# ArnauGabrielAtienza/pytorch_distributed_examples

Hardware: AMD Instinct MI355X
Metric: images/sec (whole node) MNIST DDP + ResNet50 RPC-MP at 1/2/4/8 MI355X (higher is better)
Workload: dtype bf16; 1 GPU; model=mnist_cnn_Net, global_batch=1024, image=1x28x28, parallelism=dp1, hipgraph=True, fused_step=True, rccl_nranks=1, steps_per_graph=5, allreduce=none

## Files before the change

### csrc/kernels/cnn_fused.hip

```cpp
#include <cstddef>
#include <type_traits>

#include "adasum_weights.h"
#include "common.cuh"
#include "optim_device.h"
#include "pde_kernels.h"
#include "xgmi_device.h"

namespace pde {

namespace {

constexpr int T = 1024;
constexpr int NW = T / 64;
constexpr int NI = 4;
constexpr int C1 = 10, C2 = 20, KS = 5, H0 = 28, O1 = 24, P1 = 12, O2 = 8, P2 = 4, F1 = 50, F2 = 10;
constexpr int NX = H0 * H0, NC1 = P1 * P1, NR1 = C1 * NC1, NC2 = P2 * P2, NIN = C2 * NC2;
constexpr int RP16 = 146, RP8 = 148;
static_assert(RP16 >= NC1 && RP8 >= NC1, "channel planes hold the 144 cells");
static_assert(RP16 % 2 == 0 && RP8 % 4 == 0, "P9 reads 4 cells' argmax bytes as one aligned 4-byte word");
constexpr int EP = 148;
constexpr unsigned char AM_DEAD = 0xFF;
constexpr int XP = 36, NXP = H0 * XP;
constexpr int DHP = 52;
// ... 8 lines not shown
constexpr int D2N_P = 24, D2N_RP = 264, D2N_Q = 128;
constexpr int D2N_IM = 7 * D2N_RP + 7 * D2N_P + 2 * D2N_Q + 8;
static_assert(D2N_IM % 8 == 0 && D2N_P % 8 == 0 && D2N_RP % 8 == 0 && D2N_Q % 8 == 0, "d2n: 16-byte slots");
__host__ __device__ constexpr int d2n_ofs(int im, int y, int x, int co) {
  return im * D2N_IM + y * D2N_RP + x * D2N_P + (co >> 3) * D2N_Q + (co & 7);
}
constexpr int D2R = O2 * O2 + 8;
constexpr int MT1 = O1 * O1 / 16;
constexpr int MTD = NC1 * 1 / 16;
constexpr int KSW1 = O1 * O1 / 32;
struct KsRange {
  int lo, hi;
};
__host__ __device__ constexpr bool p7b_tap_live(int cls, int r, int ky, int kx) {
  const int pos = cls * 16 + r, y = pos / P1 - ky, x = pos % P1 - kx;
  return y >= 0 && y < O2 && x >= 0 && x < O2;
}
__host__ __device__ constexpr KsRange p7b_ks_range(int cls) {
  int lo = KSD, hi = 0;
  for (int r = 0; r < 16; ++r)
    for (int ky = 0; ky < KS; ++ky)
      for (int kx = 0; kx < KS; ++kx) {
        if (!p7b_tap_live(cls, r, ky, kx)) continue;
        const int g0 = (ky * KS + kx) * CG, k0 = g0 / 4, k1 = (g0 + CG - 1) / 4;
        lo = k0 < lo ? k0 : lo;
        hi = k1 + 1 > hi ? k1 + 1 : hi;
      }
  return {lo, hi};
}
__host__ __device__ constexpr bool p7b_range_covers(int cls, KsRange q) {
  for (int g = 0; g < NGD; ++g)
    for (int r = 0; r < 16; ++r)
      if (p7b_tap_live(cls, r, g / CG / KS, g / CG % KS) && (g / 4 < q.lo || g / 4 >= q.hi)) return false;
  return q.lo >= 0 && q.hi <= KSD;
}
__host__ __device__ constexpr bool p7b_ranges_ok() {
  int sum = 0;
  for (int c = 0; c < MTD; ++c) {
    if (!p7b_range_covers(c, p7b_ks_range(c))) return false;
    sum += p7b_ks_range(c).hi - p7b_ks_range(c).lo;
  }
  return sum == 126;
}
constexpr bool ks_is(KsRange q, int lo, int hi) { return q.lo == lo && q.hi == hi; }
static_assert(MTD == 9 && NC1 % 16 == 0 && p7b_ranges_ok(), "conv2 dgrad: every live tap inside its class's range");
static_assert(ks_is(p7b_ks_range(0), 0, 7) && ks_is(p7b_ks_range(1), 0, 12) && ks_is(p7b_ks_range(2), 0, 15) &&
                  ks_is(p7b_ks_range(3), 0, KSD) && ks_is(p7b_ks_range(4), 0, KSD) &&
                  ks_is(p7b_ks_range(5), 0, KSD) && ks_is(p7b_ks_range(6), 3, KSD) &&
                  ks_is(p7b_ks_range(7), 7, KSD) && ks_is(p7b_ks_range(8), 12, KSD),
              "conv2 dgrad k-step ranges (rows 0-1, 1-2, 2-3, 4..7, 8-9, 9-10, 10-11)");
__host__ __device__ constexpr uint64_t p7b_pack(bool hi) {
  uint64_t v = 0;
  for (int c = 0; c < MTD; ++c)
    v |= static_cast<uint64_t>(hi ? p7b_ks_range(c).hi : p7b_ks_range(c).lo) << (5 * c);
  return v;
}
constexpr uint64_t P7B_LO = p7b_pack(false), P7B_HI = p7b_pack(true);
static_assert(KSD < 32 && MTD * 5 <= 64, "5-bit fields");
constexpr int P7B_WCLS[NW] = {3, 4, 5, 5, 3, 4, 6, 6, 1, 7, 2, 2, 1, 7, 0, 0};
constexpr int P7B_WPAIR[NW] = {0, 0, 0, 1, 1, 1, 0, 1, 0, 0, 0, 1, 1, 1, 0, 1};
__host__ __device__ constexpr int p7b_wave_steps(int w) {
  const int c = P7B_WCLS[w];
  int n = p7b_ks_range(c).hi - p7b_ks_range(c).lo;
  if (c == 0) n += p7b_ks_range(MTD - 1).hi - p7b_ks_range(MTD - 1).lo;
  return 2 * n;
}
__host__ __device__ constexpr bool p7b_map_ok() {
  for (int c = 0; c < MTD - 1; ++c) {
    int n[2] = {0, 0};
    for (int w = 0; w < NW; ++w)
      if (P7B_WCLS[w] == c) ++n[P7B_WPAIR[w]];
    if (n[0] != 1 || n[1] != 1) return false;
  }
  int tot = 0;
  for (int s = 0; s < 4; ++s) {
    int n = 0;
    for (int w = s; w < NW; w += 4) n += p7b_wave_steps(w);
    if (n < 120 || n > 132) return false;
    tot += n;
  }
  return tot == NI * 126;
}
static_assert(NW == 16 && NI == 4 && p7b_map_ok(), "conv2 dgrad wave map: complete, balanced over the SIMDs");
__host__ __device__ constexpr uint64_t p7b_pack_map(bool pair) {
  uint64_t v = 0;
  for (int w = 0; w < NW; ++w) v |= static_cast<uint64_t>(pair ? P7B_WPAIR[w] : P7B_WCLS[w]) << (4 * w);
  return v;
}
constexpr uint64_t P7B_MCLS = p7b_pack_map(false), P7B_MPAIR = p7b_pack_map(true);
constexpr int XMAP_P7B_FULLK = 8;
constexpr int O_W1 = 0, O_B1 = O_W1 + W1N, O_W2 = O_B1 + C1, O_B2 = O_W2 + W2N, O_FC1W = O_B2 + C2,
              O_FC1B = O_FC1W + FC1N, O_FC2W = O_FC1B + F1, O_FC2B = O_FC2W + FC2N, NPARAM = O_FC2B + F2;
constexpr int NSLAB = NPARAM - FC1N;
static_assert(O_W2 % 4 == 0 && C2 % 4 == 0 && W2N % 4 == 0, "W2T: float4 columns of 4 co");
constexpr int SLAB_OFS = (32 - O_W2 % 32) % 32;
constexpr int NSLABP = (SLAB_OFS + NSLAB + 31) / 32 * 32;
constexpr int S_FC1B = O_FC1B - FC1N, S_FC2W = O_FC2W - FC1N, S_FC2B = O_FC2B - FC1N;
constexpr int NACT = F1 + NIN;
__host__ __device__ constexpr int act_pitch(int nwg) { return (nwg * NI + 7) & ~7; }
static_assert(O_FC1W % 4 == 0 && FC1N % 4 == 0 && NSLAB % 4 == 0, "float4 slab columns");

__device__ __forceinline__ float hash_u01(unsigned long long seed, unsigned long long id) {
  unsigned long long z = seed + 0x9E3779B97F4A7C15ULL * (id + 1);
  z = (z ^ (z >> 30)) * 0xBF58476D1CE4E5B9ULL;
  z = (z ^ (z >> 27)) * 0x94D049BB133111EBULL;
  z ^= z >> 31;
  return static_cast<float>(z >> 40) * (1.0f / 16777216.0f);
}

__device__ __forceinline__ f32x4 mfma(const u16x8& a, const u16x8& b, const f32x4& c) {
  return __builtin_amdgcn_mfma_f32_16x16x32_bf16(__builtin_bit_cast(bf16x8, a), __builtin_bit_cast(bf16x8, b), c, 0,
                                                 0, 0);
}

template <int CTRL>
__device__ __forceinline__ float dppf(float v) {
  return __builtin_bit_cast(float, __builtin_amdgcn_update_dpp(0, __builtin_bit_cast(int, v), CTRL, 0xF, 0xF, false));
}
__device__ __forceinline__ float lanef(float v, int l) {
  return __builtin_bit_cast(float, __builtin_amdgcn_readlane(__builtin_bit_cast(int, v), l));
}
constexpr int DPP_XOR1 = 0xB1, DPP_XOR2 = 0x4E, DPP_HALF_MIRROR = 0x141, DPP_MIRROR = 0x140;
template <class Op>
__device__ __forceinline__ float wave_all(float v, Op op) {
  v = op(v, dppf<DPP_XOR1>(v));
  v = op(v, dppf<DPP_XOR2>(v));
  v = op(v, dppf<DPP_HALF_MIRROR>(v));
  v = op(v, dppf<DPP_MIRROR>(v));
  return op(op(lanef(v, 0), lanef(v, 16)), op(lanef(v, 32), lanef(v, 48)));
}
__device__ __forceinline__ float wave_sum_dpp(float v) { return wave_all(v, [](float a, float b) { return a + b; }); }
__device__ __forceinline__ float wave_max_dpp(float v) { return wave_all(v, [](float a, float b) { return fmaxf(a, b); }); }

struct CnnSmem {
  alignas(16) uint16_t r1n[NI][NC1][C1P];
  alignas(16) u16x8 w2f[KS2][2][64];
  alignas(16) u16x8 w2d[KSD][64];
  alignas(16) u16x8 w1f[64];
  alignas(16) uint16_t d2n[NI * D2N_IM];
  alignas(16) uint16_t d2[NI][C2][D2R];
  alignas(16) uint16_t zero16[8];
  alignas(8) uint32_t p7tab[KSD * 4][2];
  uint16_t x[NI][NXP];
  uint16_t xpad[18];
  uint16_t x1[NI][NXP];
  uint16_t xonepad[48];
  alignas(16) uint16_t xone[NI][NXP];
  alignas(16) uint16_t r1[NI][C1 * RP16];
  alignas(16) float b1[C1];
  alignas(16) float b2[C2];
  alignas(16) float fc1b[F1];
  alignas(16) float fc2w[FC2N];
  alignas(16) float fc2b[F2];
  alignas(16) float r2[NI][NIN];
  alignas(16) float dp2[NI][NIN];
  float h1[NI][F1], m1[NI][F1], h1d[NI][F1];
  alignas(16) float dh[NI][DHP];
  float mc2[NI][C2];
  float logit[NI][F2], dlog[NI][F2];
  float lossim[NI];
  float valid[NI];
  int label[NI];
  alignas(16) unsigned char a1[NI][C1 * RP8];
  unsigned char a2[NI][NIN];
};
static_assert(sizeof(CnnSmem) <= 160 * 1024, "LDS budget");
static_assert((offsetof(CnnSmem, xone) - offsetof(CnnSmem, x)) / 4 % 32 == 4,
              "xone bank offset from x (P9 B reads: scripts/p9_lds_model.py; x1's: cnn_p1)");
static_assert(offsetof(CnnSmem, w2f) == offsetof(CnnSmem, r1n) + sizeof(uint16_t) * NI * NC1 * C1P &&
                  sizeof(uint32_t) * NI * C1 * EP <= sizeof(uint16_t) * NI * NC1 * C1P + sizeof(u16x8) * KS2 * 2 * 64,
              "e1 aliases r1n + w2f");
static_assert(offsetof(CnnSmem, d2n) == offsetof(CnnSmem, w1f) + sizeof(u16x8) * 64 &&
                  NW * 2 * 64 * sizeof(f32x4) <= sizeof(u16x8) * (KSD * 64 + 64) + sizeof(uint16_t) * NI * D2N_IM,
              "P9 partials alias w2d + w1f + d2n (not e1)");
static_assert(offsetof(CnnSmem, w2d) == offsetof(CnnSmem, w2f) + sizeof(u16x8) * KS2 * 2 * 64, "w2f, w2d adjacent");
constexpr int NT2 = 16 / NW;
constexpr int NFRAG = KS2 * 2 * 64 + KSD * 64 + 64;
constexpr int NF2F = KS2 * 2 * 64, NF2D = KSD * 64;
static_assert(NF2F <= 2 * T && NF2D <= 2 * T && NF2F + NF2D + 64 == NFRAG, "fragment slots");
static_assert(offsetof(CnnSmem, w1f) == offsetof(CnnSmem, w2d) + sizeof(u16x8) * KSD * 64, "w2d, w1f adjacent");
constexpr int FC1_KC = NIN / 32;
constexpr int DP2_JC = 3;
constexpr int DP2_J = 16;
static_assert(F1 - DP2_J * (DP2_JC - 1) <= 20 && DP2_J % 4 == 0 && DHP >= DP2_J * (DP2_JC - 1) + 20, "dp2 chunks");
static_assert(F1 * FC1_KC <= T && NIN * DP2_JC <= T, "fc1 work split");
static_assert(sizeof(float) * NI * NIN * DP2_JC <= sizeof(u16x8) * KS2 * 2 * 64, "dp2 partials alias w2f");
static_assert(NT2 * NW == 16, "conv2 wgrad tiling");

__device__ __forceinline__ void lds_sync() {
  __builtin_amdgcn_fence(__ATOMIC_RELEASE, "workgroup", "local");
  __builtin_amdgcn_s_barrier();
  __builtin_amdgcn_fence(__ATOMIC_ACQUIRE, "workgroup", "local");
}

__device__ __forceinline__ uint32_t lds_addr(const void* p) {
#if defined(__HIP_DEVICE_COMPILE__)
  return (uint32_t)(const __attribute__((address_space(3))) unsigned char*)(p);
#else
  return static_cast<uint32_t>(reinterpret_cast<uintptr_t>(p));
#endif
}
__device__ __forceinline__ u16x8 lds_read16(uint32_t o) {
#if defined(__HIP_DEVICE_COMPILE__)
  return *(const __attribute__((address_space(3))) u16x8*)(o);
#else
  return u16x8{static_cast<uint16_t>(o), 0, 0, 0, 0, 0, 0, 0};
#endif
}

struct CnnTail {
  const float* gscale;
  float* grads;
  float* loss;
  unsigned long long* rng;
  float* params;
  const float* hp;
  uint16_t* frag;
  int* step;
  unsigned* bar;
  int* err;
  int accumulate, B, on, pad;
};
__device__ void cnn_fused_tail(const CnnTail& tl, int rb, f32x4* part, uint32_t* s_epoch, int* s_fail,
                               const float* slabs, int nwg, const uint16_t* acts, const float* loss_part);

__device__ __forceinline__ void cnn_grid_barrier(unsigned* bar, unsigned n, int* err, unsigned* s_gen) {
  asm volatile("s_waitcnt vmcnt(0)" ::: "memory");
  __syncthreads();
  if (threadIdx.x == 0) {
    const unsigned g0 = __hip_atomic_load(bar + 1, __ATOMIC_RELAXED, __HIP_MEMORY_SCOPE_AGENT);
    __builtin_amdgcn_fence(__ATOMIC_RELEASE, "agent");
    const unsigned old = __hip_atomic_fetch_add(bar, 1u, __ATOMIC_RELAXED, __HIP_MEMORY_SCOPE_AGENT);
    if (old == n - 1) {
      __hip_atomic_store(bar, 0u, __ATOMIC_RELAXED, __HIP_MEMORY_SCOPE_AGENT);
      __hip_atomic_fetch_add(bar + 1, 1u, __ATOMIC_RELEASE, __HIP_MEMORY_SCOPE_AGENT);
    } else {
      const uint64_t t0 = __builtin_amdgcn_s_memrealtime();
      while (__hip_atomic_load(bar + 1, __ATOMIC_RELAXED, __HIP_MEMORY_SCOPE_AGENT) == g0) {
        if (__builtin_amdgcn_s_memrealtime() - t0 > 200000000ull) {
          __hip_atomic_store(err, 1, __ATOMIC_RELAXED, __HIP_MEMORY_SCOPE_AGENT);
          break;
        }
        __builtin_amdgcn_s_sleep(1);
      }
    }
    __builtin_amdgcn_fence(__ATOMIC_ACQUIRE, "agent");
    *s_gen = g0;
  }
  __syncthreads();
}

template <int SM>
__device__ __forceinline__ void out_st(float* p, float v) {
  if constexpr (SM == 1) __builtin_nontemporal_store(v, p);
  else if constexpr (SM == 2) asm volatile("global_store_dword %0, %1, off sc1" ::"v"(p), "v"(v) : "memory");
  else *p = v;
}
template <int SM>
__device__ __forceinline__ void out_st_u16x4(uint16_t* p, u16x4 v) {
  if constexpr (SM == 1) __builtin_nontemporal_store(v, reinterpret_cast<u16x4*>(p));
  else st_vec(reinterpret_cast<u16x4*>(p), v, SM >= 2);
}
template <int SM>
__device__ __forceinline__ void out_st4(float* p, f32x4 v) {
  if constexpr (SM == 1) __builtin_nontemporal_store(v, reinterpret_cast<f32x4*>(p));
  else if constexpr (SM >= 2) asm volatile("global_store_dwordx4 %0, %1, off sc1" ::"v"(p), "v"(v) : "memory");
  else *reinterpret_cast<f32x4*>(p) = v;
}

template <bool TRAIN, class Smem>
__device__ __forceinline__ void cnn_p0(Smem& S, int t, int n0, int B, const float* __restrict__ images,
                                       const int64_t* __restrict__ tgt, const float* __restrict__ params,
                                       const u16x8* __restrict__ frag, const unsigned long long* __restrict__ rng,
                                       float p_drop2, float p_drop1, int training, u16x8 (&fr)[2]) {
  static_assert(NI * NX / 4 <= T, "one image quad per thread");
  constexpr int NH = C1 + C2 + F1 + FC2N + F2;
  static_assert(NH <= T && O_FC2W == O_FC1B + F1 && O_FC2B == O_FC2W + FC2N, "fc1b, fc2w, fc2b contiguous");
  static_assert(offsetof(Smem, fc2b) == offsetof(Smem, fc2w) + sizeof(float) * FC2N, "fc2w, fc2b adjacent");
  static_assert((NI & (NI - 1)) == 0 && 384 % NI == 0, "label threads 384..: slot t & (NI - 1)");
  const int qi = min(t, NI * NX / 4 - 1);
  const int qim = (qi * 4) / NX, qoff = qi * 4 - qim * NX;
  const int hi = min(t, NH - 1);
  const int hsrc = hi < C1 ? O_B1 + hi : hi < C1 + C2 ? O_B2 + hi - C1 : O_FC1B + hi - (C1 + C2);
  const int lslot = t & (NI - 1);
  const int64_t* lbase = tgt != nullptr ? tgt : reinterpret_cast<const int64_t*>(frag);
  const int lidx = tgt != nullptr ? min(n0 + lslot, B - 1) : 0;
  int rofs = 0;
  asm("" : "+v"(rofs));
  const u16x8 fw1 = frag[NF2F + NF2D + (t & 63)];
  const f32x4 img = *reinterpret_cast<const f32x4*>(images + static_cast<long>(min(n0 + qim, B - 1)) * NX + qoff);
  const float hv = params[hsrc];
  unsigned long long r0 = 0;
  if constexpr (TRAIN) r0 = rng[rofs];
  const int lab = reinterpret_cast<const int*>(lbase)[2 * lidx];
  fr[0] = frag[t];
  fr[1] = frag[min(t + T, NF2F - 1)];
  static_assert(H0 % 4 == 0 && XP >= H0 + 6, "image quads within a row; kx = 5 reads stay in the row");
  for (int i = t; i < NI * H0 * (XP - H0 + 1); i += T) {
    const int r = i / (XP - H0 + 1), c = i - r * (XP - H0 + 1);
    if (c > 0) (&S.x[0][0])[r * XP + H0 - 1 + c] = 0;
    (&S.x1[0][0])[r * XP + H0 - 1 + c] = 0;
  }
  if constexpr (TRAIN) {
    for (int i = t; i < NI * O2 * O2; i += T) {
      const int im = i / (O2 * O2), pos = i - im * (O2 * O2);
      *reinterpret_cast<u16x8*>(&S.d2n[d2n_ofs(im, pos / O2, pos % O2, 16)]) = u16x8{0, 0, 0, 0, 0, 0, 0, 0};
    }
    if (t < 8) S.zero16[t] = 0;
    static_assert((NI * NXP) % 8 == 0 && NI * NXP / 8 <= T, "xone: one 16-byte store per thread");
    if (t < NI * NXP / 8)
      reinterpret_cast<u16x8*>(&S.xone[0][0])[t] =
          u16x8{0x3F80, 0x3F80, 0x3F80, 0x3F80, 0x3F80, 0x3F80, 0x3F80, 0x3F80};
    if (t < KSD * 4) {
      const int g = t, tap = g / CG, cg = g - tap * CG, ky = tap / KS, kx = tap - ky * KS;
      S.p7tab[g][0] = g < NGD ? (static_cast<uint32_t>(ky) << 16) | static_cast<uint32_t>(kx) : 0x80008000u;
      S.p7tab[g][1] = static_cast<uint32_t>(g < NGD ? (-(ky * D2N_RP + kx * D2N_P) + cg * D2N_Q) * 2 : 0);
    }
  }
  if (t < 64) S.w1f[t] = fw1;
  if (t < NI * NX / 4) {
    const int im = qim, off = qoff, n = n0 + im;
    const f32x4 v = n < B ? img : f32x4{0.f, 0.f, 0.f, 0.f};
    const int row = off / H0, col = off - row * H0;
    uint16_t* dst = &S.x[im][row * XP + col];
    const uint16_t b0 = f2bf(v[0]), b1 = f2bf(v[1]), b2 = f2bf(v[2]), b3 = f2bf(v[3]);
    dst[0] = b0; dst[1] = b1; dst[2] = b2; dst[3] = b3;
    uint16_t* d1 = &S.x1[im][row * XP + col];
    if (col > 0) d1[-1] = b0;
    d1[0] = b1; d1[1] = b2; d1[2] = b3;
  }
  if (t < NH) {
    const int hofs = hi < C1             ? static_cast<int>(offsetof(Smem, b1)) + 4 * hi
                     : hi < C1 + C2      ? static_cast<int>(offsetof(Smem, b2)) + 4 * (hi - C1)
                     : hi < C1 + C2 + F1 ? static_cast<int>(offsetof(Smem, fc1b)) + 4 * (hi - (C1 + C2))
                                         : static_cast<int>(offsetof(Smem, fc2w)) + 4 * (hi - (C1 + C2 + F1));
    *reinterpret_cast<float*>(reinterpret_cast<unsigned char*>(&S) + hofs) = hv;
  }
  if constexpr (TRAIN) {
    const unsigned long long seed = r0 * 0xD1B54A32D192ED03ULL;
    const float keep2 = training ? 1.f / (1.f - p_drop2) : 1.f;
    const float keep1 = training ? 1.f / (1.f - p_drop1) : 1.f;
    if (t < NI * C2) {
      const int im = t / C2, c = t - im * C2;
      const unsigned long long id = static_cast<unsigned long long>(n0 + im) * C2 + c;
      S.mc2[im][c] = (!training || hash_u01(seed ^ 0x5bd1e995ULL, id) >= p_drop2) ? keep2 : 0.f;
    } else if (t >= 128 && t < 128 + NI * F1) {
      const int u = t - 128, im = u / F1, j = u - im * F1;
      const unsigned long long id = static_cast<unsigned long long>(n0 + im) * F1 + j;
      S.m1[im][j] = (!training || hash_u01(seed ^ 0x27d4eb2fULL, id) >= p_drop1) ? keep1 : 0.f;
    }
  }
  if (t >= 384 && t < 384 + NI) {
    const bool ok = tgt != nullptr && n0 + lslot < B;
    if constexpr (TRAIN) S.valid[lslot] = ok ? 1.f : 0.f;
    S.label[lslot] = ok ? static_cast<int>(lab) : 0;
  }
}


__device__ __forceinline__ float pool4(const f32x4& v, int& am) {
  am = 0;
  float m = v[0];
  if (v[1] > m) { m = v[1]; am = 1; }
  if (v[2] > m) { m = v[2]; am = 2; }
  if (v[3] > m) { m = v[3]; am = 3; }
  return m;
}

static_assert(P1 % 4 == 0 && MT1 * 4 == NC1, "conv1 tiles: 4 cells of one row");
static_assert((NI * MT1) % NW == 0, "every wave runs the same number of conv1 tiles");
constexpr int NT1 = NI * MT1 / NW;
constexpr int P1_TR = P1 / 4;
static_assert(MT1 % NT1 == 0, "conv1: a wave's tiles lie in one image");
static_assert(NT1 % P1_TR == 0, "conv1: a wave's tiles are whole cell rows");
constexpr int P1_WI = MT1 / NT1;
constexpr int P1_WR = NT1 / P1_TR;
struct P1Tile {
  int im, py, px0;
};
__host__ __device__ constexpr P1Tile p1_tile(int w, int u) {
  return {w / P1_WI, (w % P1_WI) * P1_WR + u / P1_TR, (u % P1_TR) * 4};
}
__host__ __device__ constexpr bool p1_map_ok() {
  for (int tile = 0; tile < NI * MT1; ++tile) {
    int n = 0;
    for (int w = 0; w < NW; ++w)
      for (int u = 0; u < NT1; ++u) {
        const P1Tile q = p1_tile(w, u);
        if (q.im < 0 || q.im >= NI || q.py < 0 || q.py >= P1 || q.px0 < 0 || q.px0 + 4 > P1) return false;
        if (q.im * MT1 + q.py * P1_TR + q.px0 / 4 == tile) ++n;
      }
    if (n != 1) return false;
  }
  return true;
}
static_assert(p1_map_ok(), "conv1 wave map: the 16 waves cover each of the NI * MT1 tiles exactly once");

template <bool TRAIN, class Smem>
__device__ __forceinline__ void cnn_p1(Smem& S, int lane, int wid) {
  static_assert((offsetof(Smem, x1) - offsetof(Smem, x)) / 4 % 32 == 9, "x1 bank offset from x (P1 gathers)");
  const int lr = lane & 15, lg = lane >> 4;
  int koff[4];
#pragma unroll
  for (int p = 0; p < 4; ++p) {
    const int k = lg * 8 + 2 * p;
    koff[p] = k < KS * 6 ? (k / 6) * XP + (k % 6) : 0;
  }
  const u16x8 bw = S.w1f[lane];
  const int tap = lr & 3, dy = tap >> 1, dx = tap & 1;
  const uint16_t* xsrc = dx ? &S.x1[0][0] - 1 : &S.x[0][0];
  const P1Tile w0 = p1_tile(wid, 0);
  const uint16_t* xlane = xsrc + dy * XP + 2 * (lr >> 2) + dx + w0.im * NXP + 2 * w0.py * XP;
  const uint16_t* xb[4];
#pragma unroll
  for (int p = 0; p < 4; ++p) xb[p] = xlane + koff[p];
  u16x8 ag[NT1];
#pragma unroll
  for (int u = 0; u < NT1; ++u) {
    const P1Tile q = p1_tile(0, u);
    const int xo = 2 * q.py * XP + 2 * q.px0;
    u32x4 v;
#pragma unroll
    for (int p = 0; p < 4; ++p) v[p] = *reinterpret_cast<const uint32_t*>(xb[p] + xo);
    ag[u] = __builtin_bit_cast(u16x8, v);
  }
  f32x4 accs[NT1];
#pragma unroll
  for (int u = 0; u < NT1; ++u) accs[u] = mfma(ag[u], bw, f32x4{0.f, 0.f, 0.f, 0.f});
  const int co = lr;
  const float b1v = S.b1[min(co, C1 - 1)];
  const float bias1 = co < C1 ? b1v : 0.f;
  const int cw = w0.py * P1 + lg;
  uint16_t* r1n = &S.r1n[w0.im][cw][co];
  uint16_t rr[NT1];
  int am[NT1];
#pragma unroll
  for (int u = 0; u < NT1; ++u) {
    const P1Tile q = p1_tile(0, u);
    const float m = pool4(accs[u], am[u]);
    rr[u] = f2bf(fmaxf(m + bias1, 0.f));
    r1n[(q.py * P1 + q.px0) * C1P] = rr[u];
    if constexpr (TRAIN) {
      if (rr[u] == 0) am[u] = AM_DEAD;
      asm volatile("" : "+v"(am[u]));
    }
  }
  if constexpr (TRAIN) {
    if (co < C1) {
      uint16_t* r1 = &S.r1[w0.im][co * RP16 + cw];
      unsigned char* a1 = &S.a1[w0.im][co * RP8 + cw];
#pragma unroll
      for (int u = 0; u < NT1; ++u) {
        const P1Tile q = p1_tile(0, u);
        r1[q.py * P1 + q.px0] = rr[u];
        a1[q.py * P1 + q.px0] = static_cast<unsigned char>(am[u]);
      }
    }
  }
}

template <class Smem>
__device__ __forceinline__ void cnn_store_w2f(Smem& S, int t, const u16x8 (&fr)[2]) {
  u16x8* dst = &S.w2f[0][0][0];
  dst[t] = fr[0];
  if (t + T < NF2F) dst[t + T] = fr[1];
}

__device__ __forceinline__ void cnn_fc1_rows(int t, const float* __restrict__ gFC1W, f32x4 (&w3)[8]) {
  if (t < F1 * FC1_KC) {
    const int j = t / FC1_KC, kc = t - j * FC1_KC;
    const f32x4* w4 = reinterpret_cast<const f32x4*>(gFC1W + j * NIN + kc * 4);
#pragma unroll
    for (int q = 0; q < 8; ++q) w3[q] = w4[q * (FC1_KC)];
  }
}

template <bool TRAIN, class Smem>
__device__ __forceinline__ void cnn_p2(Smem& S, int lane, int wid) {
  const int lr = lane & 15, lg = lane >> 4;
  for (int mtile = wid; mtile < NI * 4; mtile += NW) {
    const int im = mtile >> 2, mt = mtile & 3;
    const int tap = lr & 3, dy = tap >> 1, dx = tap & 1;
    const int cell = mt * 4 + (lr >> 2), py = cell >> 2, px = cell & 3;
    const int rb = (2 * py + dy) * P1 + 2 * px + dx;
    f32x4 acc0 = {0.f, 0.f, 0.f, 0.f}, acc1 = acc0;
    const uint16_t* r1n = &S.r1n[im][0][(lg & 1) * 8];
#pragma unroll
    for (int ks = 0; ks < KS2; ++ks) {
      const int tp = 2 * ks + (lg >> 1), ky = tp / KS, kx = tp - ky * KS;
      const u16x8 a = tp < KS * KS ? *reinterpret_cast<const u16x8*>(r1n + (rb + ky * P1 + kx) * C1P)
                                   : u16x8{0, 0, 0, 0, 0, 0, 0, 0};
      acc0 = mfma(a, S.w2f[ks][0][lane], acc0);
      acc1 = mfma(a, S.w2f[ks][1][lane], acc1);
    }
#pragma unroll
    for (int nt = 0; nt < 2; ++nt) {
      const int co = nt * 16 + lr;
      if (co < C2) {
        int am;
        const float m = pool4(nt == 0 ? acc0 : acc1, am);
        const int q = co * NC2 + mt * 4 + lg;
        if constexpr (TRAIN) {
          S.r2[im][q] = fmaxf((m + S.b2[co]) * S.mc2[im][co], 0.f);
          S.a2[im][q] = static_cast<unsigned char>(am);
        } else {
          S.r2[im][q] = fmaxf(m + S.b2[co], 0.f);
        }
      }
    }
  }
}

template <bool TRAIN, class Smem>
__device__ __forceinline__ void cnn_p3(Smem& S, int t, const f32x4 (&w3)[8]) {
  static_assert(sizeof(float) * NI * F1 * FC1_KC <= sizeof(Smem::w2f), "fc1 partials alias w2f");
  float* part = reinterpret_cast<float*>(&S.w2f[0][0][0]);
  if (t < F1 * FC1_KC) {
    const int j = t / FC1_KC, kc = t - j * FC1_KC;
    const f32x4* w = w3;
    float s4[NI] = {0.f, 0.f, 0.f, 0.f};
#pragma unroll
    for (int q = 0; q < 8; ++q)
#pragma unroll
      for (int im = 0; im < NI; ++im) {
        const f32x4 x = *reinterpret_cast<const f32x4*>(&S.r2[im][q * 4 * FC1_KC + kc * 4]);
        s4[im] += w[q][0] * x[0] + w[q][1] * x[1] + w[q][2] * x[2] + w[q][3] * x[3];
      }
#pragma unroll
    for (int im = 0; im < NI; ++im) part[(kc * NI + im) * F1 + j] = s4[im];
  }
  lds_sync();
  if (t < NI * F1) {
    const int im = t / F1, j = t - im * F1;
    float s1 = S.fc1b[j];
#pragma unroll
    for (int kc = 0; kc < FC1_KC; ++kc) s1 += part[(kc * NI + im) * F1 + j];
    const float h = fmaxf(s1, 0.f);
    S.h1[im][j] = h;
    if constexpr (TRAIN) S.h1d[im][j] = h * S.m1[im][j];
  }
}

struct CnnHead {
  float logit;
  float lse;
  float ly;
  int y;
};
template <class Smem>
__device__ __forceinline__ CnnHead cnn_head(const Smem& S, const float* h, int im, int lane) {
  static_assert(4 * F2 <= 64, "P4: a lane quad per logit");
  const int v = lane >> 2, p = lane & 3;
  const bool lv = v < F2;
  const int vr = lv ? v : 0;
  float s = 0.f;
#pragma unroll
  for (int k = 0; k < (F1 + 3) / 4; ++k) {
    const int j = p + 4 * k;
    if (j < F1) s += S.fc2w[vr * F1 + j] * h[j];
  }
  s += dppf<DPP_XOR1>(s);
  s += dppf<DPP_XOR2>(s);
  const float logit = s + S.fc2b[vr];
  const float m = wave_max_dpp(lv ? logit : -INFINITY);
  const float ex = __expf(logit - m);
  const float se = wave_sum_dpp(lv && p == 0 ? ex : 0.f);
  const float lse = m + __logf(se);
  const int y = S.label[im];
  const float ly = lanef(logit, __builtin_amdgcn_readfirstlane(4 * y));
  return {logit, lse, ly, y};
}

template <int SM, bool BREG>
__global__ __launch_bounds__(T) void k_cnn_train(const float* __restrict__ images, const int64_t* __restrict__ tgt,
                                                 int B, const float* __restrict__ params,
                                                 const u16x8* __restrict__ frag,
                                                 const unsigned long long* __restrict__ rng, float p_drop2,
                                                 float p_drop1, int training, float* __restrict__ slabs,
                                                 float* __restrict__ loss_part, uint16_t* __restrict__ acts,
                                                 unsigned long long* __restrict__ stamps, int stop_after,
                                                 CnnTail tail, int xmap) {
#define PDE_STAMP(k)                                                                      \
  if (stamps != nullptr && threadIdx.x == 0) stamps[blockIdx.x * 16 + (k)] = wall_clock64(); \
  if (stop_after == (k)) return
  asm volatile("" ::"s"(images), "s"(tgt), "s"(B), "s"(params), "s"(frag), "s"(rng), "s"(p_drop2), "s"(p_drop1),
               "s"(training), "s"(slabs), "s"(loss_part), "s"(acts), "s"(stamps), "s"(stop_after), "s"(xmap),
               "s"(tail.accumulate), "s"(tail.B), "s"(tail.on), "s"(gridDim.x));
  PDE_STAMP(0);
  extern __shared__ __attribute__((aligned(16))) unsigned char smem_raw[];
  CnnSmem& S = *reinterpret_cast<CnnSmem*>(smem_raw);
  const int t = threadIdx.x;
  const int lane = t & 63;
  const int wid = __builtin_amdgcn_readfirstlane(t >> 6);
  const int lr = lane & 15, lg = lane >> 4;
  const float* gW1 = params + O_W1;
  const float* gW2 = params + O_W2;
  const float* gFC1W = params + O_FC1W;
  const int lwg = (xmap & 1) ? (blockIdx.x & 7) * (gridDim.x >> 3) + (blockIdx.x >> 3) : blockIdx.x;
  const int n0 = lwg * NI;

  u16x8 fr[2];
  cnn_p0<true>(S, t, n0, B, images, tgt, params, frag, rng, p_drop2, p_drop1, training, fr);
  float* slab = slabs + static_cast<long>(blockIdx.x) * NSLABP + SLAB_OFS;
  lds_sync();
  PDE_STAMP(1);

  cnn_p1<true>(S, lane, wid);
  if (stamps != nullptr) {
    if (t == 0) stamps[blockIdx.x * 16 + 13] = wall_clock64();
    if (t == 15 * 64) stamps[blockIdx.x * 16 + 15] = wall_clock64();
  }
  if (!(xmap & 2)) cnn_store_w2f(S, t, fr);
  lds_sync();
  PDE_STAMP(2);

  f32x4 w3[8];
  cnn_fc1_rows(t, gFC1W, w3);
  cnn_p2<true>(S, lane, wid);
  lds_sync();
  PDE_STAMP(3);

  cnn_p3<true>(S, t, w3);
  lds_sync();
  PDE_STAMP(4);

  constexpr int JPER = F1 - DP2_J * (DP2_JC - 1);
  float w6[JPER];
  {
    const int tc = min(t, NIN * DP2_JC - 1);
    const int jc = tc / NIN, i = tc - jc * NIN;
#pragma unroll
    for (int u = 0; u < JPER; ++u) w6[u] = gFC1W[min(jc * DP2_J + u, F1 - 1) * NIN + i];
  }
  u16x8 fd[2];
  if constexpr (!BREG) {
    fd[0] = frag[NF2F + t];
    fd[1] = frag[NF2F + min(t + T, NF2D - 1)];
  }

  static_assert(NI <= NW, "P4: a wave per image");
  if (wid < NI) {
    const int im = wid, v = lane >> 2, p = lane & 3;
    const bool lv = v < F2;
    const auto [logit, lse, ly, y] = cnn_head(S, S.h1d[im], im, lane);
    const float val = S.valid[im];
    const float dl = (__expf(logit - lse) - (v == y ? 1.f : 0.f)) * val;
    if (lv && p == 0) S.dlog[im][v] = dl;
    if (lane == 0) S.lossim[im] = val * (lse - ly);
    static_assert(F1 <= 64, "P4: a lane per fc1 output");
    const int j = lane < F1 ? lane : 0;
    float sh = 0.f;
#pragma unroll
    for (int vv = 0; vv < F2; ++vv) sh += S.fc2w[vv * F1 + j] * lanef(dl, 4 * vv);
    if (lane < F1) S.dh[im][lane] = (S.h1[im][lane] > 0.f) ? sh * S.m1[im][lane] : 0.f;
  }
  lds_sync();
  PDE_STAMP(5);
  PDE_STAMP(6);
  PDE_STAMP(7);


  static_assert(FC2N + F2 <= T, "fc2 weight / bias gradients: one element per thread");
  if (t < FC2N) {
    const int v = t / F1, j = t - v * F1;
    float s = 0.f;
#pragma unroll
    for (int im = 0; im < NI; ++im) s += S.dlog[im][v] * S.h1d[im][j];
    out_st<SM>(&slab[S_FC2W + t], s);
  } else if (t < FC2N + F2) {
    const int v = t - FC2N;
    float s = 0.f;
#pragma unroll
    for (int im = 0; im < NI; ++im) s += S.dlog[im][v];
    out_st<SM>(&slab[S_FC2B + v], s);
  }
  {
    const int Bk = gridDim.x * NI, Bkp = act_pitch(gridDim.x);
    const bool pad = Bkp != Bk && n0 + NI == Bk;
    for (int row = t; row < NACT; row += T) {
      u16x4 v;
#pragma unroll
      for (int im = 0; im < NI; ++im) v[im] = f2bf(row < F1 ? S.dh[im][row] : S.r2[im][row - F1]);
      out_st_u16x4<SM>(acts + static_cast<long>(row) * Bkp + n0, v);
      if (pad) out_st_u16x4<SM>(acts + static_cast<long>(row) * Bkp + n0 + NI, u16x4{0, 0, 0, 0});
    }
  }
  if (t < F1) {
    float s = 0.f;
#pragma unroll
    for (int im = 0; im < NI; ++im) s += S.dh[im][t];
    out_st<SM>(&slab[S_FC1B + t], s);
  }
  float* dpart = reinterpret_cast<float*>(&S.w2f[0][0][0]);
  if (t < NIN * DP2_JC) {
    const int jc = t / NIN, i = t - jc * NIN;
    const int j0 = jc * DP2_J, nj = jc == DP2_JC - 1 ? F1 - j0 : DP2_J;
    const float* w = w6;
    float s4[NI] = {0.f, 0.f, 0.f, 0.f};
#pragma unroll
    for (int im = 0; im < NI; ++im)
#pragma unroll
      for (int q = 0; q < (JPER + 3) / 4; ++q) {
        const f32x4 d = *reinterpret_cast<const f32x4*>(&S.dh[im][j0 + 4 * q]);
#pragma unroll
        for (int e = 0; e < 4; ++e) {
          const int u = 4 * q + e;
          if (u < JPER) s4[im] += u < nj ? w[u] * d[e] : 0.f;
        }
      }
#pragma unroll
    for (int im = 0; im < NI; ++im) dpart[(jc * NI + im) * NIN + i] = s4[im];
  }
  lds_sync();
  for (int it = t; it < NI * NIN; it += T) {
    const int im = it / NIN, q = it - im * NIN, co = q / NC2, cell = q - co * NC2;
    float s1 = 0.f;
#pragma unroll
    for (int jc = 0; jc < DP2_JC; ++jc) s1 += dpart[(jc * NI + im) * NIN + q];
    const float v = (S.r2[im][q] > 0.f) ? s1 * S.mc2[im][co] : 0.f;
    S.dp2[im][q] = v;
    const int py = cell >> 2, px = cell & 3, a = S.a2[im][q];
    const uint16_t g = f2bf(v);
    const int p00 = (2 * py) * O2 + 2 * px;
    const uint32_t gv = g;
    *reinterpret_cast<uint32_t*>(&S.d2[im][co][p00]) = a == 0 ? gv : (a == 1 ? gv << 16 : 0u);
    *reinterpret_cast<uint32_t*>(&S.d2[im][co][p00 + O2]) = a == 2 ? gv : (a == 3 ? gv << 16 : 0u);
    uint16_t* dn = &S.d2n[d2n_ofs(im, 2 * py, 2 * px, co)];
    dn[0] = a == 0 ? g : 0;
    dn[D2N_P] = a == 1 ? g : 0;
    dn[D2N_RP] = a == 2 ? g : 0;
    dn[D2N_RP + D2N_P] = a == 3 ? g : 0;
  }
  if constexpr (!BREG) {
    u16x8* dst = &S.w2d[0][0];
    dst[t] = fd[0];
    if (t + T < NF2D) dst[t + T] = fd[1];
  }
  lds_sync();
  PDE_STAMP(8);
  if (t >= 448 && t < 448 + C2) {
    const int co = t - 448;
    f32x4 s4 = {0.f, 0.f, 0.f, 0.f};
#pragma unroll
    for (int im = 0; im < NI; ++im)
#pragma unroll
      for (int c = 0; c < NC2; c += 4) s4 += *reinterpret_cast<const f32x4*>(&S.dp2[im][co * NC2 + c]);
    out_st<SM>(&slab[O_B2 + co], (s4[0] + s4[1]) + (s4[2] + s4[3]));
  }
  constexpr int KSB = 8;
  u16x8 bd[BREG ? KSD : 1];
  if constexpr (BREG) {
#pragma unroll
    for (int ks = 0; ks < KSB; ++ks) bd[ks] = frag[NF2F + ks * 64 + lane];
  }

  {
    int nb[NT2];
#pragma unroll
    for (int u = 0; u < NT2; ++u) {
      const int kidx = (wid * NT2 + u) * 16 + lr, ci = kidx / 25, r = kidx - ci * 25, ky = r / 5, kx = r - ky * 5;
      nb[u] = kidx < K2 ? ci * RP16 + ky * P1 + kx : 0;
    }
    const uint16_t* arow[2];
#pragma unroll
    for (int mt = 0; mt < 2; ++mt) arow[mt] = &S.d2[0][min(mt * 16 + lr, C2 - 1)][0];
    f32x4 acc[2][NT2];
#pragma unroll
    for (int u = 0; u < NT2; ++u) acc[0][u] = acc[1][u] = f32x4{0.f, 0.f, 0.f, 0.f};
    for (int ks = 0; ks < KSW2; ++ks) {
      const int im = ks >> 1, y = (ks & 1) * 4 + lg;
      u16x8 a[2];
#pragma unroll
      for (int mt = 0; mt < 2; ++mt) a[mt] = *reinterpret_cast<const u16x8*>(arow[mt] + im * C2 * D2R + y * O2);
#pragma unroll
      for (int u = 0; u < NT2; ++u) {
        const int e0 = nb[u] + y * P1;
        const uint32_t* wp = reinterpret_cast<const uint32_t*>(&S.r1[im][0]) + (e0 >> 1);
        const uint32_t sh = static_cast<uint32_t>(e0 & 1) * 2;
        uint32_t w[5];
#pragma unroll
        for (int q = 0; q < 5; ++q) w[q] = wp[q];
        u32x4 v;
#pragma unroll
        for (int q = 0; q < 4; ++q) v[q] = __builtin_amdgcn_alignbyte(w[q + 1], w[q], sh);
        const u16x8 b = __builtin_bit_cast(u16x8, v);
        acc[0][u] = mfma(a[0], b, acc[0][u]);
        acc[1][u] = mfma(a[1], b, acc[1][u]);
      }
    }
#pragma unroll
    for (int mt = 0; mt < 2; ++mt)
#pragma unroll
      for (int u = 0; u < NT2; ++u) {
        const int kidx = (wid * NT2 + u) * 16 + lr, cg = mt * 4 + lg;
        if (cg * 4 < C2 && kidx < K2) out_st4<SM>(&slab[O_W2 + (cg * K2 + kidx) * 4], acc[mt][u]);
      }
  }
  PDE_STAMP(9);

  {
    constexpr int MAXT = 2;
    const int cls0 = static_cast<int>(P7B_MCLS >> (4 * wid)) & 15;
    const int im0 = (static_cast<int>(P7B_MPAIR >> (4 * wid)) & 1) * MAXT;
    const int npass = cls0 == 0 ? 2 : 1;
    const bool fullk = BREG || (xmap & XMAP_P7B_FULLK) != 0;
    const uint32_t sbase = lds_addr(smem_raw);
    const uint32_t zpo = sbase + static_cast<uint32_t>(offsetof(CnnSmem, zero16));
    constexpr uint32_t IMB = D2N_IM * 2;
    uint32_t* e1 = reinterpret_cast<uint32_t*>(&S.r1n[0][0][0]);
    auto run_pass = [&](int pass) {
      const int cls = pass == 0 ? cls0 : MTD - 1;
      const int lo = fullk ? 0 : static_cast<int>(P7B_LO >> (5 * cls)) & 31;
      const int hi = fullk ? KSD : static_cast<int>(P7B_HI >> (5 * cls)) & 31;
      const int pos = cls * 16 + lr, ty = pos / P1, tx = pos - ty * P1;
      const u16x2 tyx{static_cast<uint16_t>(tx), static_cast<uint16_t>(ty)};
      const uint32_t tpo = sbase + static_cast<uint32_t>(offsetof(CnnSmem, d2n)) + d2n_ofs(im0, ty, tx, 0) * 2;
      f32x4 acc[MAXT];
#pragma unroll
      for (int u = 0; u < MAXT; ++u) acc[u] = f32x4{0.f, 0.f, 0.f, 0.f};
      const int ci = lr, cell = cls * 16 + lg * 4;
      uint32_t am4[MAXT];
#pragma unroll
      for (int u = 0; u < MAXT; ++u)
        am4[u] = *reinterpret_cast<const uint32_t*>(&S.a1[im0 + u][min(ci, C1 - 1) * RP8 + cell]);

      auto tab = [&](int ks) { return *reinterpret_cast<const u32x2*>(&S.p7tab[min(ks, KSD - 1) * 4 + lg][0]); };
      auto load = [&](const u32x2& e, u16x8 (&a)[MAXT]) {
        const u16x2 kyx = __builtin_bit_cast(u16x2, e[0]);
        const bool ok = (__builtin_bit_cast(uint32_t, static_cast<u16x2>(tyx - kyx)) & 0xFFF8FFF8u) == 0u;
        const uint32_t src = tpo + e[1];
#pragma unroll
        for (int u = 0; u < MAXT; ++u) {
          uint32_t o = ok ? src + u * IMB : zpo;
          asm("" : "+v"(o));
          a[u] = lds_read16(o);
        }
      };
      if constexpr (BREG) {
        u16x8 an[MAXT];
        load(tab(0), an);
        u32x2 en = tab(1);
#pragma unroll
        for (int ks = 0; ks < KSD; ++ks) {
          u16x8 ac[MAXT];
#pragma unroll
          for (int u = 0; u < MAXT; ++u) ac[u] = an[u];
          if (ks + KSB < KSD) bd[ks + KSB] = frag[NF2F + (ks + KSB) * 64 + lane];
          if (ks + 1 < KSD) {
            const u32x2 e = en;
            en = tab(ks + 2);
            load(e, an);
          }
#pragma unroll
          for (int u = 0; u < MAXT; ++u) acc[u] = mfma(ac[u], bd[ks], acc[u]);
        }
        if (pass + 1 < npass) {
#pragma unroll
          for (int ks = 0; ks < KSB; ++ks) bd[ks] = frag[NF2F + ks * 64 + lane];
        }
      } else {
        u16x8 ae[MAXT], ao[MAXT], be, bo;
        load(tab(lo), ae);
        be = S.w2d[lo][lane];
        u32x2 en = tab(lo + 1);
        int ks = lo;
        for (; ks + 2 < hi; ks += 2) {
          u32x2 e = en;
          en = tab(ks + 2);
          load(e, ao);
          bo = S.w2d[ks + 1][lane];
#pragma unroll
          for (int u = 0; u < MAXT; ++u) acc[u] = mfma(ae[u], be, acc[u]);
          e = en;
          en = tab(ks + 3);
          load(e, ae);
          be = S.w2d[ks + 2][lane];
#pragma unroll
          for (int u = 0; u < MAXT; ++u) acc[u] = mfma(ao[u], bo, acc[u]);
        }
        if (ks + 1 < hi) {
          load(en, ao);
          bo = S.w2d[ks + 1][lane];
#pragma unroll
          for (int u = 0; u < MAXT; ++u) acc[u] = mfma(ae[u], be, acc[u]);
#pragma unroll
          for (int u = 0; u < MAXT; ++u) acc[u] = mfma(ao[u], bo, acc[u]);
        } else {
#pragma unroll
          for (int u = 0; u < MAXT; ++u) acc[u] = mfma(ae[u], be, acc[u]);
        }
      }
      if (ci < C1) {
#pragma unroll
        for (int u = 0; u < MAXT; ++u) {
          const int im = im0 + u;
          u32x4 e;
#pragma unroll
          for (int r = 0; r < 4; ++r) {
            const uint32_t am = (am4[u] >> (8 * r)) & 0xFFu;
            e[r] = am == AM_DEAD ? 0u : static_cast<uint32_t>(f2bf(acc[u][r])) << (16 * (am & 1u));
          }
          *reinterpret_cast<u32x4*>(&e1[(im * C1 + ci) * EP + cell]) = e;
        }
      }
    };
    if constexpr (BREG) {
      run_pass(0);
      if (npass > 1) run_pass(1);
    } else {
      for (int pass = 0; pass < npass; ++pass) run_pass(pass);
    }
  }
  lds_sync();
  PDE_STAMP(10);

  {
    const uint16_t* xw[2];
#pragma unroll
    for (int u = 0; u < 2; ++u) {
      const int k0 = u * 16 + lr, kidx = k0 > 25 ? 17 : k0;
      const int nb = (kidx / 5) * XP + kidx % 5;
      xw[u] = kidx == 25 ? &S.xone[0][0] : ((kidx % 5) & 1 ? &S.x1[0][0] - 1 : &S.x[0][0]) + nb;
    }
    f32x4 acc[2] = {f32x4{0.f, 0.f, 0.f, 0.f}, f32x4{0.f, 0.f, 0.f, 0.f}};
    const int co = lr;
    const int cr = co < C1 ? co : 0;
    const uint32_t* e1 = reinterpret_cast<const uint32_t*>(&S.r1n[0][0][0]);
    constexpr int NK9 = (NI * KSW1 + NW - 1) / NW;
    static_assert(KSW1 * 4 * 2 == NC1 && P1 % 2 == 0, "P9: 4 lane groups x 2 cells per k-step");
    uint32_t m9[NK9];
    u32x2 e9[NK9];
    u16x8 b9[NK9][2];
#pragma unroll
    for (int u9 = 0; u9 < NK9; ++u9) {
      const int ks = wid + u9 * NW;
      if (ks >= NI * KSW1) break;
      const int im = ks / KSW1;
      const uint32_t gi = static_cast<uint32_t>((ks - im * KSW1) * 4 + lg);
      const uint32_t py = (gi * 43u) >> 8, pc = gi - py * 6u;
      const int cell = static_cast<int>(py * P1 + pc * 2);
      m9[u9] = *reinterpret_cast<const uint16_t*>(&S.a1[im][cr * RP8 + cell]);
      e9[u9] = *reinterpret_cast<const u32x2*>(&e1[(im * C1 + cr) * EP + cell]);
      const int off = im * NXP + static_cast<int>(py * 2 * XP + pc * 4);
#pragma unroll
      for (int u = 0; u < 2; ++u) {
        const uint16_t* src = xw[u] + off;
        u32x4 v;
        v[0] = *reinterpret_cast<const uint32_t*>(src);
        v[1] = *reinterpret_cast<const uint32_t*>(src + 2);
        v[2] = *reinterpret_cast<const uint32_t*>(src + XP);
        v[3] = *reinterpret_cast<const uint32_t*>(src + XP + 2);
        b9[u9][u] = __builtin_bit_cast(u16x8, v);
      }
    }
#pragma unroll
    for (int u9 = 0; u9 < NK9; ++u9) {
      if (wid + u9 * NW >= NI * KSW1) break;
      u32x4 a;
#pragma unroll
      for (int c = 0; c < 2; ++c) {
        const bool lower = (m9[u9] >> (8 * c + 1)) & 1u;
        a[c] = lower ? 0u : e9[u9][c];
        a[2 + c] = lower ? e9[u9][c] : 0u;
      }
#pragma unroll
      for (int u = 0; u < 2; ++u) acc[u] = mfma(__builtin_bit_cast(u16x8, a), b9[u9][u], acc[u]);
    }
    f32x4* part = reinterpret_cast<f32x4*>(&S.w2d[0][0]);
    part[(wid * 2 + 0) * 64 + lane] = acc[0];
    part[(wid * 2 + 1) * 64 + lane] = acc[1];
    lds_sync();
    if (stamps != nullptr && t == 0) stamps[blockIdx.x * 16 + 14] = wall_clock64();
    static_assert(O_W1 == 0 && O_B1 == W1N && (W1N + C1) % 4 == 0, "conv1 gradients: one float4 run");
    if (wid * 64 < W1N + C1) {
      const bool live = t < W1N + C1;
      const int c = t < W1N ? t / 25 : (live ? t - W1N : 0);
      const int kidx = t < W1N ? t - c * 25 : 25;
      const int u = kidx >> 4;
      const int l = (c >> 2) * 16 + (kidx & 15), r = c & 3;
      float s = 0.f;
#pragma unroll
      for (int w = 0; w < NW; ++w) s += part[(w * 2 + u) * 64 + l][r];
      const int si = __builtin_bit_cast(int, s);
      const f32x4 q{s, __builtin_bit_cast(float, __builtin_amdgcn_update_dpp(0, si, 0x55, 0xF, 0xF, false)),
                    __builtin_bit_cast(float, __builtin_amdgcn_update_dpp(0, si, 0xAA, 0xF, 0xF, false)),
                    __builtin_bit_cast(float, __builtin_amdgcn_update_dpp(0, si, 0xFF, 0xF, 0xF, false))};
      if (live && (t & 3) == 0 && !(xmap & 4))
        out_st4<SM>(&slab[O_W1 + t], q);
    }
  }
  PDE_STAMP(11);

  if (wid == 0) {
    const float l = wave_sum_dpp(lane < NI ? S.lossim[lane] : 0.f);
    if (lane == 0) out_st<SM>(&loss_part[blockIdx.x], l);
  }
  if (stamps != nullptr) {
    asm volatile("s_waitcnt vmcnt(0)" ::: "memory");
    __syncthreads();
    PDE_STAMP(12);
  }
  if (tail.on) {
    __shared__ uint32_t s_epoch;
    __shared__ int s_fail;
    __shared__ unsigned s_gen;
    cnn_grid_barrier(tail.bar, gridDim.x, tail.err, &s_gen);
    cnn_fused_tail(tail, blockIdx.x, reinterpret_cast<f32x4*>(&S.w2f[0][0][0]), &s_epoch, &s_fail, slabs,
                   gridDim.x, acts, loss_part);
  }
}

__global__ __launch_bounds__(256) void k_cnn_prep(const float* __restrict__ params, u16x8* __restrict__ frag) {
  const int e = blockIdx.x * 256 + threadIdx.x;
  if (e >= NFRAG) return;
  const float* gW1 = params + O_W1;
  const float* gW2 = params + O_W2;
  u16x8 f;
  if (e < KS2 * 2 * 64) {
    const int ks = e >> 7, nt = (e >> 6) & 1, l = e & 63;
    const int co = nt * 16 + (l & 15), g = l >> 4, tap = 2 * ks + (g >> 1), c8 = (g & 1) * 8;
#pragma unroll
    for (int j = 0; j < 8; ++j)
      f[j] = (co < C2 && tap < KS * KS && c8 + j < C1) ? f2bf(gW2[co * K2 + (c8 + j) * KS * KS + tap]) : 0;
  } else if (e < KS2 * 2 * 64 + KSD * 64) {
    const int e2 = e - KS2 * 2 * 64, ks = e2 >> 6, l = e2 & 63;
    const int ci = l & 15, g = ks * 4 + (l >> 4), tap = g / CG, c0 = (g - tap * CG) * 8;
#pragma unroll
    for (int j = 0; j < 8; ++j)
      f[j] = (g < NGD && ci < C1 && c0 + j < C2) ? f2bf(gW2[(c0 + j) * K2 + ci * 25 + tap]) : 0;
  } else {
    const int l = e - KS2 * 2 * 64 - KSD * 64;
    const int co = l & 15, k0 = (l >> 4) * 8;
#pragma unroll
    for (int j = 0; j < 8; ++j) {
      const int k = k0 + j, ky = k / 6, kx = k - ky * 6;
      f[j] = (co < C1 && k < KS * 6 && kx < KS) ? f2bf(gW1[co * 25 + ky * KS + kx]) : 0;
    }
  }
  frag[e] = f;
// ... 889 lines not shown
```

Before: 41.69 million images/s.

## Rebalance backward LDS work across waves and sparsify pool-grad scatter

Zeroes the d2n and d2 planes together with flat 16-byte stores up front, then scatters only the single argmax gradient per pool cell instead of writing all four slots. The r1 plane is no longer written in the forward pool epilogue; idle waves rebuild it from r1n and stage the w2d fragments while the head waves compute the loss. The dpart partial sums move before the fc2 gradient stores, and the dp2 scatter handles two images per thread in one pass. The aim is to shorten the critical path between barriers, at the cost of more complex indexing and a dependence on the shared-memory layout holding d2n and d2 adjacent.

```diff
diff --git a/csrc/kernels/cnn_fused.hip b/csrc/kernels/cnn_fused.hip
--- a/csrc/kernels/cnn_fused.hip
+++ b/csrc/kernels/cnn_fused.hip
@@ -334,9 +334,17 @@
     (&S.x1[0][0])[r * XP + H0 - 1 + c] = 0;
   }
   if constexpr (TRAIN) {
-    for (int i = t; i < NI * O2 * O2; i += T) {
-      const int im = i / (O2 * O2), pos = i - im * (O2 * O2);
-      *reinterpret_cast<u16x8*>(&S.d2n[d2n_ofs(im, pos / O2, pos % O2, 16)]) = u16x8{0, 0, 0, 0, 0, 0, 0, 0};
+    constexpr int NZ = (sizeof(Smem::d2n) + sizeof(Smem::d2)) / 16;
+    static_assert(offsetof(Smem, d2) == offsetof(Smem, d2n) + sizeof(Smem::d2n) && sizeof(Smem::d2n) % 16 == 0 &&
+                      sizeof(Smem::d2) % 16 == 0 && NZ > T && NZ <= 2 * T,
+                  "d2n, d2 adjacent: two 16-byte stores per thread");
+    static_assert(sizeof(Smem::d2n) == sizeof(uint16_t) * NI * D2N_IM &&
+                      d2n_ofs(NI - 1, O2 - 1, O2 - 1, CG * 8 - 1) == NI * D2N_IM - 1 && d2n_ofs(0, 0, 0, 0) == 0,
+                  "d2n: the zeroed extent is first to last slot of (image, y, x, co < 24)");
+    {
+      u16x8* z = reinterpret_cast<u16x8*>(&S.d2n[0]);
+      z[t] = u16x8{0, 0, 0, 0, 0, 0, 0, 0};
+      if (t + T < NZ) z[t + T] = u16x8{0, 0, 0, 0, 0, 0, 0, 0};
     }
     if (t < 8) S.zero16[t] = 0;
     static_assert((NI * NXP) % 8 == 0 && NI * NXP / 8 <= T, "xone: one 16-byte store per thread");
@@ -479,12 +487,10 @@
   }
   if constexpr (TRAIN) {
     if (co < C1) {
-      uint16_t* r1 = &S.r1[w0.im][co * RP16 + cw];
       unsigned char* a1 = &S.a1[w0.im][co * RP8 + cw];
 #pragma unroll
       for (int u = 0; u < NT1; ++u) {
         const P1Tile q = p1_tile(0, u);
-        r1[q.py * P1 + q.px0] = rr[u];
         a1[q.py * P1 + q.px0] = static_cast<unsigned char>(am[u]);
       }
     }
@@ -656,6 +662,16 @@
   lds_sync();
   PDE_STAMP(4);
 
+  constexpr int TW = T - NI * 64;
+  static_assert(NF2D > TW && NF2D <= 2 * TW, "w2d: two fragment slots per thread of the waves past the heads");
+  const int iw = t - NI * 64;
+  u16x8 fd[2];
+  if constexpr (!BREG) {
+    if (wid >= NI) {
+      fd[0] = frag[NF2F + iw];
+      fd[1] = frag[NF2F + min(iw + TW, NF2D - 1)];
+    }
+  }
   constexpr int JPER = F1 - DP2_J * (DP2_JC - 1);
   float w6[JPER];
   {
@@ -663,11 +679,6 @@
     const int jc = tc / NIN, i = tc - jc * NIN;
 #pragma unroll
     for (int u = 0; u < JPER; ++u) w6[u] = gFC1W[min(jc * DP2_J + u, F1 - 1) * NIN + i];
-  }
-  u16x8 fd[2];
-  if constexpr (!BREG) {
-    fd[0] = frag[NF2F + t];
-    fd[1] = frag[NF2F + min(t + T, NF2D - 1)];
   }
 
   static_assert(NI <= NW, "P4: a wave per image");
@@ -685,6 +696,27 @@
 #pragma unroll
     for (int vv = 0; vv < F2; ++vv) sh += S.fc2w[vv * F1 + j] * lanef(dl, 4 * vv);
     if (lane < F1) S.dh[im][lane] = (S.h1[im][lane] > 0.f) ? sh * S.m1[im][lane] : 0.f;
+  } else {
+    static_assert(NC1 % 2 == 0 && RP16 % 2 == 0 && C1 > 8 && C1 <= 10 && C1P == 16 && NI * NC1 <= TW,
+                  "r1 from r1n: cell pairs as aligned words, channels 0..7 | 8, 9");
+    if (iw < NI * NC1) {
+      const uint32_t uw = static_cast<uint32_t>(iw);
+      const uint32_t im = uw / NC1, cp = (uw - im * NC1) >> 1, h = uw & 1;
+      const uint32_t* src = reinterpret_cast<const uint32_t*>(&S.r1n[0][0][0]) + (uw >> 1) * C1P + h * 4;
+      const u32x4 ev = *reinterpret_cast<const u32x4*>(src), od = *reinterpret_cast<const u32x4*>(src + C1P / 2);
+      uint32_t* dst = reinterpret_cast<uint32_t*>(&S.r1[im][0]) + h * 8 * (RP16 / 2) + cp;
+#pragma unroll
+      for (int d = 0; d < 4; ++d)
+        if (d == 0 || h == 0) {
+          dst[(2 * d) * (RP16 / 2)] = (ev[d] & 0xFFFFu) | (od[d] << 16);
+          dst[(2 * d + 1) * (RP16 / 2)] = (ev[d] >> 16) | (od[d] & 0xFFFF0000u);
+        }
+    }
+    if constexpr (!BREG) {
+      u16x8* dst = &S.w2d[0][0];
+      dst[iw] = fd[0];
+      if (iw + TW < NF2D) dst[iw + TW] = fd[1];
+    }
   }
   lds_sync();
   PDE_STAMP(5);
@@ -692,6 +724,29 @@
   PDE_STAMP(7);
 
 
+  float* dpart = reinterpret_cast<float*>(&S.w2f[0][0][0]);
+  {
+    const int tc = min(t, NIN * DP2_JC - 1);
+    const int jc = tc / NIN, i = tc - jc * NIN;
+    const int j0 = jc * DP2_J, nj = jc == DP2_JC - 1 ? F1 - j0 : DP2_J;
+    const float* w = w6;
+    float s4[NI] = {0.f, 0.f, 0.f, 0.f};
+#pragma unroll
+    for (int im = 0; im < NI; ++im)
+#pragma unroll
+      for (int q = 0; q < (JPER + 3) / 4; ++q) {
+        const f32x4 d = *reinterpret_cast<const f32x4*>(&S.dh[im][j0 + 4 * q]);
+#pragma unroll
+        for (int e = 0; e < 4; ++e) {
+          const int u = 4 * q + e;
+          if (u < JPER) s4[im] += u < nj ? w[u] * d[e] : 0.f;
+        }
+      }
+    if (t < NIN * DP2_JC) {
+#pragma unroll
+      for (int im = 0; im < NI; ++im) dpart[(jc * NI + im) * NIN + i] = s4[im];
+    }
+  }
   static_assert(FC2N + F2 <= T, "fc2 weight / bias gradients: one element per thread");
   if (t < FC2N) {
     const int v = t / F1, j = t - v * F1;
@@ -723,50 +778,50 @@
     for (int im = 0; im < NI; ++im) s += S.dh[im][t];
     out_st<SM>(&slab[S_FC1B + t], s);
   }
-  float* dpart = reinterpret_cast<float*>(&S.w2f[0][0][0]);
-  if (t < NIN * DP2_JC) {
-    const int jc = t / NIN, i = t - jc * NIN;
-    const int j0 = jc * DP2_J, nj = jc == DP2_JC - 1 ? F1 - j0 : DP2_J;
-    const float* w = w6;
-    float s4[NI] = {0.f, 0.f, 0.f, 0.f};
-#pragma unroll
-    for (int im = 0; im < NI; ++im)
-#pragma unroll
-      for (int q = 0; q < (JPER + 3) / 4; ++q) {
-        const f32x4 d = *reinterpret_cast<const f32x4*>(&S.dh[im][j0 + 4 * q]);
-#pragma unroll
-        for (int e = 0; e < 4; ++e) {
-          const int u = 4 * q + e;
-          if (u < JPER) s4[im] += u < nj ? w[u] * d[e] : 0.f;
-        }
-      }
-#pragma unroll
-    for (int im = 0; im < NI; ++im) dpart[(jc * NI + im) * NIN + i] = s4[im];
-  }
   lds_sync();
-  for (int it = t; it < NI * NIN; it += T) {
-    const int im = it / NIN, q = it - im * NIN, co = q / NC2, cell = q - co * NC2;
-    float s1 = 0.f;
-#pragma unroll
-    for (int jc = 0; jc < DP2_JC; ++jc) s1 += dpart[(jc * NI + im) * NIN + q];
-    const float v = (S.r2[im][q] > 0.f) ? s1 * S.mc2[im][co] : 0.f;
-    S.dp2[im][q] = v;
-    const int py = cell >> 2, px = cell & 3, a = S.a2[im][q];
-    const uint16_t g = f2bf(v);
-    const int p00 = (2 * py) * O2 + 2 * px;
-    const uint32_t gv = g;
-    *reinterpret_cast<uint32_t*>(&S.d2[im][co][p00]) = a == 0 ? gv : (a == 1 ? gv << 16 : 0u);
-    *reinterpret_cast<uint32_t*>(&S.d2[im][co][p00 + O2]) = a == 2 ? gv : (a == 3 ? gv << 16 : 0u);
-    uint16_t* dn = &S.d2n[d2n_ofs(im, 2 * py, 2 * px, co)];
-    dn[0] = a == 0 ? g : 0;
-    dn[D2N_P] = a == 1 ? g : 0;
-    dn[D2N_RP] = a == 2 ? g : 0;
-    dn[D2N_RP + D2N_P] = a == 3 ? g : 0;
-  }
-  if constexpr (!BREG) {
-    u16x8* dst = &S.w2d[0][0];
-    dst[t] = fd[0];
-    if (t + T < NF2D) dst[t + T] = fd[1];
+  constexpr int IH = NI / 2;
+  static_assert(NI % 2 == 0 && IH * NIN <= T, "dp2 scatter: two images per thread, one trip");
+  if (t < IH * NIN) {
+    const int im0 = t / NIN, q = t - im0 * NIN, co = q / NC2, cell = q - co * NC2;
+    const int py = cell >> 2, px = cell & 3;
+    float pj[2][DP2_JC], rv[2], mk[2];
+    int am[2];
+#pragma unroll
+    for (int u = 0; u < 2; ++u) {
+      const int im = im0 + u * IH;
+#pragma unroll
+      for (int jc = 0; jc < DP2_JC; ++jc) pj[u][jc] = dpart[(jc * NI + im) * NIN + q];
+      rv[u] = S.r2[im][q];
+      mk[u] = S.mc2[im][co];
+      am[u] = S.a2[im][q];
+    }
+#pragma unroll
+    for (int u = 0; u < 2; ++u) {
+#pragma unroll
+      for (int jc = 0; jc < DP2_JC; ++jc) asm volatile("" : "+v"(pj[u][jc]));
+      asm volatile("" : "+v"(rv[u]), "+v"(mk[u]), "+v"(am[u]));
+    }
+    float v[2];
+    uint32_t o2[2], on[2];
+#pragma unroll
+    for (int u = 0; u < 2; ++u) {
+      const int im = im0 + u * IH;
+      float s1 = 0.f;
+#pragma unroll
+      for (int jc = 0; jc < DP2_JC; ++jc) s1 += pj[u][jc];
+      v[u] = rv[u] > 0.f ? s1 * mk[u] : 0.f;
+      S.dp2[im][q] = v[u];
+      const int y = 2 * py + (am[u] >> 1), x = 2 * px + (am[u] & 1);
+      o2[u] = static_cast<uint32_t>((im * C2 + co) * D2R + y * O2 + x);
+      on[u] = static_cast<uint32_t>(d2n_ofs(im, y, x, co));
+    }
+#pragma unroll
+    for (int u = 0; u < 2; ++u)
+      if (rv[u] > 0.f) {
+        const uint16_t g = f2bf(v[u]);
+        (&S.d2[0][0][0])[o2[u]] = g;
+        S.d2n[on[u]] = g;
+      }
   }
   lds_sync();
   PDE_STAMP(8);
```

Result: faster. 42.54 million images/s (median of 6 runs) (+2.0%).
